# TinfoilHat0/Defending-Against-Backdoors-with-Robust-Learning-Rate

Measured on NVIDIA H100. Metric: fl_rounds_per_sec, higher is better.
Workload: dtype bf16

## Files before the change

defending-against-backdoors-with-robust-learning-rate_b200/models/native.py:

```python
from __future__ import annotations

import math
import os

import torch
import torch.nn.functional as F

from .. import ops
from .graph import FlatLayout

ACT = torch.bfloat16
FUSE_DROPOUT = bool(int(os.environ.get("RLR_FUSE_DROPOUT", "1")))
FUSE_RELU_POOL = bool(int(os.environ.get("RLR_FUSE_RELU_POOL", "1")))
EPILOGUE_BN_STATS = bool(int(os.environ.get("RLR_EPILOGUE_BN_STATS", "0")))
FWD_BRANCH = bool(int(os.environ.get("RLR_FWD_BRANCH", "1")))
BWD_BRANCH = bool(int(os.environ.get("RLR_BWD_BRANCH", "1")))
EPI_STAT_SLOTS = min(16, max(1, int(os.environ.get("RLR_EPI_STAT_SLOTS", "2"))))
FWD_SLOTS = BWD_SLOTS = max(1, int(os.environ.get("RLR_BN_SLOTS", "1")))
WGRAD_OVERLAP = bool(int(os.environ.get("RLR_WGRAD_OVERLAP", "1")))


def dropout_stream_base(seed: int, agent_id: int, rnd: int) -> int:
    z = (int(seed) * 0x9E3779B97F4A7C15 + (int(agent_id) + 1) * 0xBF58476D1CE4E5B9 + (int(rnd) + 1) * 0x94D049BB133111EB) & (2 ** 64 - 1)
    z = ((z ^ (z >> 30)) * 0xBF58476D1CE4E5B9) & (2 ** 64 - 1)
# ... 206 lines not shown
            op.saved["mean_rstd"] = torch.zeros(2, c, dtype=torch.float32, device=dev)
            off += 2 * c
        for op in self.plan:
            if op.kind == "gn":
                op.saved["mean_rstd"] = torch.zeros(B, 2, op.attrs["groups"], dtype=torch.float32, device=dev)
            if op.kind == "maxpool":
                op.saved["idx"] = torch.empty((B, *op.out_shape), dtype=torch.uint8, device=dev)
                if "drop" in op.saved and self.impl["pool"] != "sm100":
                    op.saved["dmask"] = torch.ones((B, *op.out_shape), dtype=torch.uint8, device=dev)
            if op.kind == "dropout":
                op.saved["mask"] = torch.empty((B, *op.out_shape), dtype=torch.uint8, device=dev)
        self._bn_src = {}
        for i, op in enumerate(self.plan):
            if not (FWD_BRANCH and op.kind == "conv" and ".downsample." in (op.name or "")):
                continue
            nxt = self.plan[i + 1] if i + 1 < len(self.plan) else None
            first = next((q for q in self.plan[:i] if q.x == op.x and q is not op), None)
            join = next((q for q in self.plan[i + 1:] if nxt is not None and q.res == nxt.y), None)
            if nxt is None or nxt.kind not in ("bn", "gn") or nxt.x != op.y or first is None or join is None:
                continue
            first.saved["fork_before"] = True
            op.saved["side_branch"] = nxt.saved["side_branch"] = True
            join.saved["join_before"] = True
        for i, op in enumerate(self.plan):
            if op.kind == "bn":
                prod = next((q for q in self.plan[:i] if q.y == op.x and q.kind == "conv"), None)
                op.saved["producer"] = prod

    def bind(self, w, wb, g, w_buffers=None):
        self.w, self.wb, self.g = w, wb, g
        lay = self.layout
        self.pw = {p.name: lay.view(w, p) for p in lay.params}
        self.pw.update({b.name: lay.view(w if w_buffers is None else w_buffers, b) for b in lay.buffers})
        self.pwb = {p.name: lay.view(wb, p) for p in lay.params} if wb is not None else {}
        self.pg = {p.name: lay.view(g, p) for p in lay.params} if g is not None else {}

    def T(self, t, B):
        return self.act[t][:B] if t != self.in_tid else self._x

    def stem_geometry(self):
        op = self.plan[0]
        if op.kind != "conv" or op.x != self.in_tid or self.impl["conv_fwd"] != "sm100" or self.impl["conv_wgrad"] != "sm100":
            return None
        return ops.stem_geometry(op.in_shape, op.attrs)

    def G(self, t, B):
# ... 92 lines not shown
        a = op.attrs
        x, y, dy = self.T(op.x, B), self.T(op.y, B), self.G(op.y, B)
        if op.relu and not op.saved.get("relu_bwd_fused"):
            ops.relu_bwd_(dy, y, self.impl["bn"])
        name = op.name + ".weight"
        gw, gb = self.pg[name], self.pg.get(op.name + ".bias")
        s, p = a.get("stride", 1), a.get("pad", 0)
        if self.impl["conv_wgrad"] == "sm100" and ops.conv_supported(op.in_shape, a, "wgrad"):
            if getattr(self, "_side", None) is not None:
                self._side.wait_stream(torch.cuda.current_stream(self.device))
                with torch.cuda.stream(self._side):
                    ops.conv2d_wgrad_sm100(x, dy, gw, gb, s, p, tag=(id(self), op.name), zero=False)
            else:
                ops.conv2d_wgrad_sm100(x, dy, gw, gb, s, p, tag=(id(self), op.name), zero=False)
        else:
            if self.impl["conv_wgrad"] == "sm100":
                ops.note_fallback("conv_wgrad", f"{op.name} in={op.in_shape} {a}")
            _, dw, db = torch.ops.aten.convolution_backward(
                dy.permute(0, 3, 1, 2), x.permute(0, 3, 1, 2), self.pwb[name].permute(0, 3, 1, 2),
                [a["cout"]] if gb is not None else None, [s, s], [p, p], [1, 1], False, [0, 0], 1, [False, True, gb is not None])
            gw.copy_(dw.permute(0, 2, 3, 1))
            if gb is not None:
                gb.copy_(db)
        if not op.need_dx:
            return
        dx = self.G(op.x, B)
        if self.impl["conv_dgrad"] == "sm100" and ops.conv_supported(op.in_shape, a, "dgrad"):
            ops.conv2d_dgrad_sm100(dy, self.pwb[name], dx, s, p, op.acc_dx)
            return
        if self.impl["conv_dgrad"] == "sm100":
            ops.note_fallback("conv_dgrad", f"{op.name} in={op.in_shape} {a}")
        di, _, _ = torch.ops.aten.convolution_backward(
            dy.permute(0, 3, 1, 2), x.permute(0, 3, 1, 2), self.pwb[name].permute(0, 3, 1, 2), None, [s, s], [p, p], [1, 1],
            False, [0, 0], 1, [True, False, False])
        di = di.permute(0, 2, 3, 1)
        if op.acc_dx:
            dx.add_(di)
        else:
            dx.copy_(di)

    def _fwd_bn(self, op, B, train):
        a = op.attrs
        x, y = self.T(op.x, B), self.T(op.y, B)
        res = self.T(op.res, B) if op.res is not None else None
        gamma, beta = self.pw[op.name + ".weight"], self.pw[op.name + ".bias"]
        rm, rv = self.pw[op.name + ".running_mean"], self.pw[op.name + ".running_var"]
        prod = op.saved["producer"]
        stats = prod.saved["stats"] if (train and prod is not None and prod.saved.get("stats_done")) else None
        if stats is not None and not self.fuse_bn_stats:
            stats = stats[0:EPI_STAT_SLOTS]
        count = x.numel() // x.shape[-1]
# ... 226 lines not shown
```

defending-against-backdoors-with-robust-learning-rate_b200/ops/__init__.py:

```python
from __future__ import annotations

import importlib.util
import os
import threading

import torch

_HERE = os.path.dirname(os.path.abspath(__file__))
_SO = os.path.join(_HERE, "_C.so")
_ext = None
_ext_err = None
_lock = threading.Lock()

MODE_IDS = {"avg": 0, "comed": 1, "sign": 2}
MAX_FUSED_AGENTS = 1024


class _Counter:
    calls = 0


class _CountingExt:
    def __init__(self, mod):
        self._mod = mod
# ... 356 lines not shown
        dl = dl.to(logits.dtype)
        if dlogits is not None:
            dlogits.copy_(dl)
            dl = dlogits
    if loss_sum is None:
        loss_sum = torch.zeros(1)
    loss_sum += loss
    if correct is not None:
        correct += (lf.argmax(1) == labels).sum().to(correct.dtype)
    return loss_sum, dl


def eval_metrics(logits, labels, loss_sum, confusion):
    if logits.is_cuda:
        ext().eval_metrics(logits.contiguous(), labels, loss_sum, confusion)
        return
    lf = logits.float()
    loss_sum += torch.nn.functional.cross_entropy(lf, labels, reduction="sum").double()
    C = lf.shape[1]
    pred = lf.argmax(1)
    confusion.view(-1).index_add_(0, labels * C + pred, torch.ones_like(labels))


from .nn import (avgpool_bwd, avgpool_fwd, bn_bwd, bn_fwd, conv2d_dgrad_sm100, conv2d_fwd_sm100, conv2d_wgrad_sm100, conv_supported,
                 dropout_bwd, dropout_fwd, gn_bwd, gn_fwd, linear_bwd, linear_fused_dropout_ok, linear_fwd, maxpool2_bwd, maxpool2_fwd, relu_bwd_, scratch, stem_geometry, STAT_SLOTS)
```

defending-against-backdoors-with-robust-learning-rate_b200/ops/csrc/gemm.cu:

```cuda
#include <cuda.h>
#include <stdlib.h>

#include "common.cuh"
#include "gemm.h"
#include "stem_gather.cuh"
#include "wgmma.cuh"

namespace rlr {

using namespace wg;

constexpr int BM = 128;
constexpr int BK = 64;
constexpr int kConsumers = 256;
constexpr int kThreads = kConsumers + 64;
constexpr int kEpiThreads = kConsumers;

template <int BN, int kOcc = 2>
struct TileCfg {
    static constexpr int kStages = kOcc == 3 ? (BN == 64 ? 3 : 2) : (BN == 64 ? 4 : 3);
    static constexpr int kABytes = BM * BK * 2;
    static constexpr int kBBytes = BN * BK * 2;
    static constexpr int kStageBytes = kABytes + kBBytes;
    static constexpr int kPitch = BN * 2 + 16;
// ... 246 lines not shown
                uint4 val = *reinterpret_cast<const uint4*>(staging + r * Cfg::kPitch + ch * 16);
                if (p.accumulate) {
                    const __nv_bfloat162* o2 = reinterpret_cast<const __nv_bfloat162*>(&oldv[j]);
                    __nv_bfloat162* v2 = reinterpret_cast<__nv_bfloat162*>(&val);
#pragma unroll
                    for (int q = 0; q < 4; ++q) {
                        const float2 a = __bfloat1622float2(v2[q]), b = __bfloat1622float2(o2[q]);
                        v2[q] = __floats2bfloat162_rn(a.x + b.x, a.y + b.y);
                    }
                }
                *reinterpret_cast<uint4*>(out + (size_t)gi * p.ldc + col0 + ch * 8) = val;
            }
        }
        if (kStats) {
            named_bar(1, kEpiThreads);
            for (int i = et; i < 2 * BN; i += kEpiThreads)
                if (col0 + (i % BN) < p.N)
                    atomicAdd(p.stats + (size_t)(blockIdx.x % kStatSlots) * 2 * p.N + (i < BN ? 0 : p.N) + col0 + (i % BN), red[i]);
        }
        }
    }
}

typedef CUresult (*EncodeTiledFn)(CUtensorMap*, CUtensorMapDataType, cuuint32_t, void*, const cuuint64_t*, const cuuint64_t*,
                                  const cuuint32_t*, const cuuint32_t*, CUtensorMapInterleave, CUtensorMapSwizzle,
                                  CUtensorMapL2promotion, CUtensorMapFloatOOBfill);

static EncodeTiledFn get_encode_fn() {
    static EncodeTiledFn fn = nullptr;
    if (!fn) {
        void* f = nullptr;
        cudaDriverEntryPointQueryResult q;
        if (cudaGetDriverEntryPoint("cuTensorMapEncodeTiled", &f, cudaEnableDefault, &q) != cudaSuccess || !f) return nullptr;
        fn = reinterpret_cast<EncodeTiledFn>(f);
    }
    return fn;
}

cudaError_t make_tmap_bf16(CUtensorMap* map, const void* base, int rank, const uint64_t* dims, const uint64_t* strides_bytes,
                           const uint32_t* box, const uint32_t* elem_strides = nullptr) {
    EncodeTiledFn fn = get_encode_fn();
    if (!fn) return cudaErrorNotSupported;
    cuuint64_t gd[5], gs[4];
    cuuint32_t bx[5], es[5];
    for (int i = 0; i < rank; ++i) {
        gd[i] = dims[i];
// ... 204 lines not shown
        const uint64_t d[4] = {(uint64_t)Cin, (uint64_t)Win, (uint64_t)Hin, (uint64_t)planes * NB};
        const uint64_t s[3] = {(uint64_t)Cin * 2, (uint64_t)Win * Cin * 2, (uint64_t)Hin * Win * Cin * 2};
        const uint32_t b[4] = {BK, (uint32_t)TW, (uint32_t)TH, (uint32_t)TN};
        const uint32_t es[4] = {1, (uint32_t)in_stride, (uint32_t)in_stride, 1};
        RLR_CUDA_CHECK(make_tmap_bf16(&tmA, x, 4, d, s, b, in_stride > 1 ? es : nullptr));
    }
    if (wtap) {
        if (bias) return cudaErrorInvalidValue;
        p.b_mn = 1; p.wcols = Cout;
        for (int t = 0; t < ntaps; ++t) p.wtap[t] = wtap[t];
        const uint64_t cols = (uint64_t)w_taps_total * Cout;
        const uint64_t d[2] = {cols, (uint64_t)Cin}, s[1] = {cols * 2};
        const uint32_t b[2] = {64, BK};
        RLR_CUDA_CHECK(make_tmap_bf16(&tmB, w, 2, d, s, b));
    } else {
        const uint64_t K = (uint64_t)ntaps * Cin;
        const uint64_t d[2] = {K, (uint64_t)Cout}, s[1] = {K * 2};
        const uint32_t b[2] = {BK, (uint32_t)bn};
        RLR_CUDA_CHECK(make_tmap_bf16(&tmB, w, 2, d, s, b));
    }
    return bn == 128 ? launch_bn<128>(tmA, tmB, p, m_tiles, st) : launch_bn<64>(tmA, tmB, p, m_tiles, st);
}

}
```

defending-against-backdoors-with-robust-learning-rate_b200/ops/csrc/gemm.h:

```cpp
#pragma once
#include <cuda_runtime.h>
#include <cuda_bf16.h>
#include <stdint.h>

#include "dropspec.h"

namespace rlr {

constexpr int kStatSlots = 16;

struct ConvGemmParams {
    int M, N, num_kb;
    int mode;
    int cblocks;
    int TW, TH, TN;
    int Ho, Wo, NB;
    int tiles_w, tiles_h;
    int ntaps;
    int in_stride;
    int out_stride, out_ph, out_pw, OutH, OutW;
    int8_t dh[9], dw[9];
    int dn[9];
    int b_mn;
    int wtap[9];
    int wcols;
    DropSpec drop;
    int tma_store;
    int split_prod;
    long long* dbg;
    const __nv_bfloat16* b_src;
    int b_ld, b_kvalid;
    const uint32_t* wait_flags;
    int wait_lo, wait_hi;
    const uint32_t* wait_epoch;
    void* out;
    int ldc;
    const float* bias;
    float* stats;
    int stat_slots;
    int relu, accumulate;
};

cudaError_t launch_gemm_bf16(const void* A, const void* B, void* out, int M, int N, int K, int lda, int ldb, int ldc,
                             const float* bias, int relu, int accumulate, float* stats, cudaStream_t st, const DropSpec* drop = nullptr);
cudaError_t launch_stem_gemm_bf16(const void* A, const void* W, void* out, int M, int N, int kvalid, int ldw, const float* bias, int relu,
                                  float* stats, const uint32_t* wait_flags, int wait_lo, int wait_hi, const uint32_t* wait_epoch,
                                  cudaStream_t st);
void set_pdl(int on);
cudaError_t launch_gemm_splitk_bf16(const void* A, const void* B, void* out, float* ws, int M, int N, int K, const float* bias, int relu,
                                    int num_sms, cudaStream_t st, const DropSpec* drop = nullptr);
void set_persistent_conv(int on);
void set_conv_occ3(int level);
void set_conv_tma_store(int on);
void set_conv_split_producer(int on);
void set_conv_trace(long long* buf);
long long* conv_trace_buf();
cudaError_t launch_conv_bf16(const void* x, const void* w, void* out, int NB, int planes, int Hin, int Win, int Cin, int Ho, int Wo,
                             int Cout, int ldc, int ntaps, const int* dh, const int* dw, const int* dplane, const float* bias,
                             int relu, int accumulate, float* stats, cudaStream_t st, const int* wtap = nullptr, int w_taps_total = 0,
                             int in_stride = 1, int out_stride = 1, int out_ph = 0, int out_pw = 0);

cudaError_t launch_conv3x3_halo_bf16(const void* x, const void* w, void* out, int NB, int Hin, int Win, int H, int W, int Cout, const float* bias,
                                     int relu, int accumulate, float* stats, int bo_mode, long long* dbg, int num_sms, cudaStream_t st);

cudaError_t launch_conv3x3_halo3_bf16(const void* x, const void* w, void* out, int NB, int H, int W, int Cout, const float* bias, int relu,
                                      int accumulate, int num_sms, cudaStream_t st);

cudaError_t launch_conv_wgrad_bf16(const void* dy, const void* x, float* dW, int NB, int planes, int Hin, int Win, int Cin, int Cin_valid,
                                   int Ho, int Wo, int Cout, int ntaps, const int* dh, const int* dw, const int* dplane, int num_sms,
                                   cudaStream_t st, int in_stride = 1);
cudaError_t launch_conv_wgrad_halo_bf16(const void* dy, const void* x, float* dW, int NB, int H, int W, int Cin_valid, int Cout,
                                        int num_sms, cudaStream_t st);
cudaError_t launch_linear_wgrad_bf16(const void* dy, const void* x, float* dW, int B, int N, int K, int num_sms, cudaStream_t st);

cudaError_t launch_ordered_sum_f32(float* out, const float* part, int nparts, long long n, cudaStream_t st);
cudaError_t launch_ordered_sum_f64(double* out, const double* part, int nparts, long long n, cudaStream_t st);
cudaError_t launch_channel_stats(const __nv_bfloat16* x, long long M, int C, float* stats , int num_sms, cudaStream_t st,
                                 int only_sum = 0, int nslots = 1);
cudaError_t launch_bn_finalize(const float* stats, int slots, float* mean_rstd, float* running_mean, float* running_var, int C,
                               float count, float eps, float momentum, int train, cudaStream_t st);
cudaError_t launch_bn_apply(const __nv_bfloat16* x, const __nv_bfloat16* res, __nv_bfloat16* y, const float* gamma, const float* beta,
                            float* mean_rstd, long long M, int C, int relu, int fin_mode, const float* stats, int slots, float count,
                            float eps, float momentum, float* running_mean, float* running_var, int num_sms, cudaStream_t st);
// ... 40 lines not shown
```

defending-against-backdoors-with-robust-learning-rate_b200/ops/csrc/gemm_binding.cpp:

```cpp
#include <torch/extension.h>
#include <ATen/cuda/CUDAContext.h>
#include <c10/cuda/CUDAGuard.h>
#include <c10/cuda/CUDAStream.h>
#include <c10/cuda/CUDACachingAllocator.h>

#include <vector>

#include "gemm.h"

namespace rlr {
void* scratch_alloc(size_t bytes, cudaStream_t st) {
    return c10::cuda::CUDACachingAllocator::raw_alloc_with_stream(bytes < 256 ? 256 : bytes, st);
}
void scratch_free(void* p) { c10::cuda::CUDACachingAllocator::raw_delete(p); }
}

namespace {
inline cudaStream_t cur_stream() { return c10::cuda::getCurrentCUDAStream().stream(); }
inline int num_sms() { return at::cuda::getCurrentDeviceProperties()->multiProcessorCount; }
inline void check(cudaError_t e, const char* what) { TORCH_CHECK(e == cudaSuccess, what, ": ", cudaGetErrorString(e)); }
template <typename T>
inline T* opt(const c10::optional<at::Tensor>& t) { return t.has_value() && t->defined() ? reinterpret_cast<T*>(t->data_ptr()) : nullptr; }
inline const __nv_bfloat16* bf(const at::Tensor& t) {
    TORCH_CHECK(t.is_cuda() && t.scalar_type() == at::kBFloat16 && t.is_contiguous(), "expected contiguous CUDA bf16 tensor");
// ... 64 lines not shown
    const int M = A.size(0), K = A.size(1), N = B.size(0);
    TORCH_CHECK(B.size(1) == K && out.size(0) == M && out.size(1) == N && ws.numel() == (int64_t)M * N);
    check(rlr::launch_gemm_splitk_bf16(bf(A), bf(B), bfm(out), f32(ws), M, N, K, opt<const float>(bias), relu, num_sms(), cur_stream(),
                                       drop.thr ? &drop : nullptr), "gemm_splitk_bf16");
}

void conv_bf16_strided(at::Tensor x, at::Tensor w, at::Tensor out, std::vector<int64_t> dh, std::vector<int64_t> dw,
                       c10::optional<at::Tensor> bias, bool relu, bool accumulate, std::vector<int64_t> wtap, int64_t w_taps_total,
                       int64_t in_stride, int64_t out_stride, int64_t out_ph, int64_t out_pw) {
    c10::cuda::CUDAGuard g(x.device());
    TORCH_CHECK(x.dim() == 4 && out.dim() == 4 && w.dim() == 2 && x.size(0) == out.size(0));
    TORCH_CHECK(out.size(1) % out_stride == 0 && out.size(2) % out_stride == 0, "output image must be a multiple of out_stride");
    const int NB = x.size(0), Hin = x.size(1), Win = x.size(2), Cin = x.size(3), Cout = out.size(3);
    const int Ho = out.size(1) / out_stride, Wo = out.size(2) / out_stride;
    const int T = (int)dh.size();
    const bool bmn = !wtap.empty();
    TORCH_CHECK(bmn ? (w.size(0) == Cin && w.size(1) == w_taps_total * Cout && (int)wtap.size() == T)
                    : (w.size(0) == Cout && w.size(1) == (int64_t)T * Cin), "filter shape");
    int a[9], b[9], c[9] = {0}, wt[9];
    for (int t = 0; t < T; ++t) { a[t] = (int)dh[t]; b[t] = (int)dw[t]; wt[t] = bmn ? (int)wtap[t] : 0; }
    check(rlr::launch_conv_bf16(bf(x), bf(w), bfm(out), NB, 1, Hin, Win, Cin, Ho, Wo, Cout, Cout, T, a, b, c, opt<const float>(bias), relu,
                                accumulate, nullptr, cur_stream(), bmn ? wt : nullptr, (int)w_taps_total, (int)in_stride, (int)out_stride,
                                (int)out_ph, (int)out_pw), "conv_bf16_strided");
}

void conv3x3_halo_bf16(at::Tensor x, at::Tensor w, at::Tensor out, c10::optional<at::Tensor> bias, bool relu, bool accumulate,
                       c10::optional<at::Tensor> stats, int64_t bo_mode, c10::optional<at::Tensor> dbg) {
    c10::cuda::CUDAGuard g(x.device());
    TORCH_CHECK(x.dim() == 4 && x.size(3) == 64 && out.dim() == 4 && w.dim() == 2 && w.size(1) == 9 * 64 && w.size(0) == out.size(3));
    TORCH_CHECK(out.size(0) == x.size(0) && out.size(1) - x.size(1) == out.size(2) - x.size(2), "halo conv: output = input + 2*pad - 2, pad in {0,1,2}");
    TORCH_CHECK(!stats.has_value() || !stats->defined() || stats->numel() == (int64_t)rlr::kStatSlots * 2 * out.size(3), "stats must be [STAT_SLOTS,2,Cout]");
    check(rlr::launch_conv3x3_halo_bf16(bf(x), bf(w), bfm(out), x.size(0), x.size(1), x.size(2), out.size(1), out.size(2), out.size(3), opt<const float>(bias), relu,
                                        accumulate, opt<float>(stats), (int)bo_mode, opt<long long>(dbg), num_sms(), cur_stream()), "conv3x3_halo_bf16");
}

void conv3x3_halo3_bf16(at::Tensor x, at::Tensor w, at::Tensor out, c10::optional<at::Tensor> bias, bool relu, bool accumulate) {
    c10::cuda::CUDAGuard g(x.device());
    TORCH_CHECK(x.dim() == 4 && x.size(3) == 64 && out.dim() == 4 && w.dim() == 2 && w.size(1) == 9 * 64 && w.size(0) == out.size(3));
    TORCH_CHECK(out.size(0) == x.size(0) && out.size(1) == x.size(1) && out.size(2) == x.size(2));
    check(rlr::launch_conv3x3_halo3_bf16(bf(x), bf(w), bfm(out), x.size(0), x.size(1), x.size(2), out.size(3), opt<const float>(bias), relu,
                                         accumulate, num_sms(), cur_stream()), "conv3x3_halo3_bf16");
}

void conv_wgrad_bf16(at::Tensor dy, at::Tensor x, at::Tensor dW, int64_t NB, int64_t planes, int64_t cin_valid, std::vector<int64_t> dh,
                     std::vector<int64_t> dw, std::vector<int64_t> dplane) {
    c10::cuda::CUDAGuard g(x.device());
// ... 216 lines not shown
    check(rlr::launch_linear_small_bwd2(bf(x), bf(dy), bf(w), const_cast<__nv_bfloat16*>(bfo(dx)), (float*)dw.data_ptr(), opt<float>(db),
                                        x.size(0), x.size(1), w.size(0), accumulate_dx, cur_stream()), "linear_small_bwd2");
}
}

void register_gemm_bindings(py::module_& m) {
    m.attr("STAT_SLOTS") = rlr::kStatSlots;
    m.def("set_persistent_conv", [](bool on) { rlr::set_persistent_conv(on ? 1 : 0); });
    m.def("set_pdl", [](bool on) { rlr::set_pdl(on ? 1 : 0); });
    m.def("set_conv_occ3", [](int64_t level) { rlr::set_conv_occ3((int)level); });
    m.def("set_conv_tma_store", [](bool on) { rlr::set_conv_tma_store(on ? 1 : 0); });
    m.def("set_conv_split_producer", [](bool on) { rlr::set_conv_split_producer(on ? 1 : 0); });
    m.def("set_conv_trace", [](c10::optional<at::Tensor> buf) {
        rlr::set_conv_trace(buf.has_value() && buf->defined() ? reinterpret_cast<long long*>(buf->data_ptr<int64_t>()) : nullptr);
    });
    m.def("gemm_bf16", &gemm_bf16, py::arg("A"), py::arg("B"), py::arg("out"), py::arg("bias"), py::arg("relu"), py::arg("accumulate"), py::arg("stats"),
          py::arg("drop_p") = 0.0, py::arg("drop_seed") = 0, py::arg("drop_step") = py::none(), py::arg("drop_stream") = 0);
    m.def("stem_gemm_bf16", &stem_gemm_bf16, py::arg("A"), py::arg("W"), py::arg("out"), py::arg("bias"), py::arg("relu"), py::arg("stats"),
          py::arg("ready_ptr") = 0, py::arg("lo") = 0, py::arg("hi") = 0, py::arg("epoch") = py::none());
    m.def("gemm_splitk_bf16", &gemm_splitk_bf16, py::arg("A"), py::arg("B"), py::arg("out"), py::arg("ws"), py::arg("bias"), py::arg("relu"),
          py::arg("drop_p") = 0.0, py::arg("drop_seed") = 0, py::arg("drop_step") = py::none(), py::arg("drop_stream") = 0);
    m.def("conv_bf16", &conv_bf16);
    m.def("conv_bf16_strided", &conv_bf16_strided);
    m.def("conv_wgrad_bf16_strided", &conv_wgrad_bf16_strided);
    m.def("conv3x3_halo_bf16", &conv3x3_halo_bf16);
    m.def("conv3x3_halo3_bf16", &conv3x3_halo3_bf16);
    m.def("conv_wgrad_bf16", &conv_wgrad_bf16);
    m.def("linear_wgrad_bf16", &linear_wgrad_bf16);
    m.def("conv_wgrad_halo_bf16", &conv_wgrad_halo_bf16);
    m.def("channel_stats", &channel_stats);
    m.def("ordered_sum", &ordered_sum);
    m.def("bias_grad", &bias_grad);
    m.def("bn_finalize", &bn_finalize);
    m.def("bn_apply", &bn_apply);
    m.def("bn_bwd", &bn_bwd);
    m.def("bn_bwd_recompute", &bn_bwd_recompute);
    m.def("gn_fwd", &gn_fwd);
    m.def("gn_bwd", &gn_bwd);
    m.def("relu_bwd", &relu_bwd, py::arg("dy"), py::arg("y"), py::arg("scale") = 1.0);
    m.def("maxpool2_fwd", &maxpool2_fwd, py::arg("x"), py::arg("y"), py::arg("idx"), py::arg("drop_p") = 0.0, py::arg("drop_seed") = 0,
          py::arg("drop_step") = py::none(), py::arg("drop_stream") = 0);
    m.def("maxpool2_bwd", &maxpool2_bwd, py::arg("dy"), py::arg("idx"), py::arg("dx"), py::arg("drop_p") = 0.0, py::arg("drop_seed") = 0,
          py::arg("drop_step") = py::none(), py::arg("drop_stream") = 0, py::arg("relu_out") = py::none());
    m.def("avgpool_fwd", &avgpool_fwd);
    m.def("avgpool_bwd", &avgpool_bwd);
    m.def("dropout_fwd", &dropout_fwd);
// ... 12 lines not shown
```

defending-against-backdoors-with-robust-learning-rate_b200/ops/nn.py:

```python
from __future__ import annotations

import math
import os

import torch
import torch.nn.functional as F

_scratch = {}
_s2d_done = {}
STAT_SLOTS = 16
USE_WGRAD_HALO = True
USE_STRIDED_TMA = bool(int(os.environ.get("RLR_STRIDED_TMA", "1")))
USE_IM2COL_STEM = bool(int(os.environ.get("RLR_IM2COL_STEM", "1")))
USE_BN_RECOMPUTE = bool(int(os.environ.get("RLR_BN_RECOMPUTE", "1")))
USE_HALO3 = bool(int(os.environ.get("RLR_HALO3", "0")))
USE_HALO_ANY = bool(int(os.environ.get("RLR_HALO_ANY", "1")))
USE_SPLITK = bool(int(os.environ.get("RLR_SPLITK", "1")))
USE_HEAD_V2 = bool(int(os.environ.get("RLR_HEAD_V2", "1")))


def _stem_ok(k, stride, cin, cout):
    return USE_IM2COL_STEM and stride == 1 and cin * k * k <= 64 and cout % 8 == 0 and (cout <= 64 or cout % 128 == 0)


def stem_geometry(in_shape, a):
    h, w, c = in_shape
    k, s, p = a["k"], a.get("stride", 1), a.get("pad", 0)
    if not _stem_ok(k, s, c, a["cout"]):
        return None
    return k, p, h + 2 * p - k + 1, w + 2 * p - k + 1


def _ext():
    from . import ext
    return ext()
# ... 121 lines not shown
    B = dy.shape[0]
    if stride == 2:
        return _conv2d_dgrad_s2(e, dy, w, dx, pad, accumulate)
    if _halo_ok(k, 1, k - 1 - pad, Cout, dy.shape[1], dy.shape[2]) and dx.shape[-1] % 8 == 0:
        wt = scratch(("wt", w.data_ptr(), dx.data_ptr()), (Cin, k * k * Cout), w.dtype, w.device)
        e.filter_transpose(w, wt, Cout, k * k, Cin)
        if USE_HALO3 and pad == 1 and dy.shape[1] % 16 == 0:
            e.conv3x3_halo3_bf16(dy, wt, dx, None, False, bool(accumulate))
        else:
            e.conv3x3_halo_bf16(dy, wt, dx, None, False, bool(accumulate), None, 0, None)
        return dx
    dh, dw, pl = _taps(k, 1, k - 1 - pad)
    if Cin % 64 == 0:
        T = k * k
        e.conv_bf16(dy, w.reshape(Cout, T * Cin), dx, B, 1, dh, dw, pl, None, False, bool(accumulate), None,
                    [T - 1 - t for t in range(T)], T)
        return dx
    wt = scratch(("wt", w.data_ptr(), dx.data_ptr()), (Cin, k * k * Cout), w.dtype, w.device)
    e.filter_transpose(w, wt, Cout, k * k, Cin)
    e.conv_bf16(dy, wt, dx, B, 1, dh, dw, pl, None, False, bool(accumulate), None, [], 0)
    return dx


def _conv2d_dgrad_s2(e, dy, w, dx, pad, accumulate):
    Cout, k, _, Cin = w.shape
    B, Ho, Wo, _ = dy.shape
    plan = []
    for pi in range(2):
        for pj in range(2):
            taps, dh, dw = [], [], []
            for fy in range(k):
                for fx in range(k):
                    if (pi + pad - fy) % 2 == 0 and (pj + pad - fx) % 2 == 0:
                        taps.append(fy * k + fx); dh.append((pi + pad - fy) // 2); dw.append((pj + pad - fx) // 2)
            if taps:
                plan.append((pi, pj, taps, dh, dw))
    if USE_STRIDED_TMA and Cin % 64 == 0 and dx.shape[1] == 2 * Ho and dx.shape[2] == 2 * Wo:
        if not accumulate and len(plan) < 4:
            _zero(dx)
        for pi, pj, taps, dh, dw in plan:
            e.conv_bf16_strided(dy, w.reshape(Cout, k * k * Cin), dx, dh, dw, None, False, bool(accumulate), taps, k * k, 1, 2, pi, pj)
        return dx
    dx4 = scratch(("dx4", w.data_ptr(), dx.data_ptr()), (4 * B, Ho, Wo, Cin), dy.dtype, dy.device)
    mask = 0
    for pi, pj, taps, dh, dw in plan:
        plane = pi * 2 + pj
        mask |= 1 << plane
        if Cin % 64 == 0:
            e.conv_bf16(dy, w.reshape(Cout, k * k * Cin), dx4[plane * B:(plane + 1) * B], B, 1, dh, dw, [0] * len(taps), None,
                        False, False, None, taps, k * k)
            continue
        wt = scratch(("wt_s2", w.data_ptr(), dx.data_ptr(), plane), (Cin, len(taps) * Cout), w.dtype, w.device)
        e.filter_gather_transpose(w, wt, Cout, k * k, Cin, taps)
        e.conv_bf16(dy, wt, dx4[plane * B:(plane + 1) * B], B, 1, dh, dw, [0] * len(taps), None, False, False, None, [], 0)
    e.depth_to_space(dx4, dx, bool(accumulate), mask)
    return dx


def conv2d_wgrad_sm100(x, dy, gw, gb, stride, pad, tag="fwd", zero=True):
# ... 323 lines not shown
```

Baseline: 0.5344.

## Fuse stride-2 dgrad planes and downsample shortcut dgrad into one kernel

Adds a single-launch UMMA kernel that computes all four output parity planes of a stride-2 conv dgrad at once, instead of one launch per plane plus a zeroing pass. For ResNet downsample blocks, the 1x1 stride-2 shortcut conv's dgrad is folded into the main conv's kernel as extra K-blocks on the (0,0) plane, so the separate shortcut launch and its read-modify-write accumulation disappear. The plan builder marks these pairs and skips the shortcut's own dgrad. The cost is added complexity, tensor map setup per call, and a shortcut partial that is rounded to bf16 before it is summed in.

```diff
diff --git a/defending-against-backdoors-with-robust-learning-rate_b200/models/native.py b/defending-against-backdoors-with-robust-learning-rate_b200/models/native.py
--- a/defending-against-backdoors-with-robust-learning-rate_b200/models/native.py
+++ b/defending-against-backdoors-with-robust-learning-rate_b200/models/native.py
@@ -252,6 +252,20 @@
             first.saved["fork_before"] = True
             op.saved["side_branch"] = nxt.saved["side_branch"] = True
             join.saved["join_before"] = True
+        if self.impl["conv_dgrad"] == "sm100" and ops.nn.USE_FUSED_S2_DGRAD and ops.nn.USE_STRIDED_TMA:
+            for i, op in enumerate(self.plan):
+                if not (op.kind == "conv" and ".downsample." in (op.name or "")) or not op.need_dx or op.acc_dx or op.relu:
+                    continue
+                first = next((q for q in self.plan[:i] if q.kind == "conv" and q.x == op.x), None)
+                writers = [q for q in self.plan if q.x == op.x or q.res == op.x]
+                a = op.attrs
+                if (first is None or len(writers) != 2 or (a["k"], a.get("stride", 1), a.get("pad", 0)) != (1, 2, 0)
+                        or first.attrs.get("stride", 1) != 2 or first.attrs["cout"] != a["cout"]
+                        or not ops.conv_supported(first.in_shape, first.attrs, "dgrad") or not ops.conv_supported(op.in_shape, a, "dgrad")):
+                    continue
+                first.saved["dgrad_shortcut"] = op
+                op.saved["dgrad_folded"] = True
+                first.acc_dx = False
         for i, op in enumerate(self.plan):
             if op.kind == "bn":
                 prod = next((q for q in self.plan[:i] if q.y == op.x and q.kind == "conv"), None)
@@ -390,11 +404,15 @@
             gw.copy_(dw.permute(0, 2, 3, 1))
             if gb is not None:
                 gb.copy_(db)
-        if not op.need_dx:
+        if not op.need_dx or op.saved.get("dgrad_folded"):
             return
         dx = self.G(op.x, B)
         if self.impl["conv_dgrad"] == "sm100" and ops.conv_supported(op.in_shape, a, "dgrad"):
-            ops.conv2d_dgrad_sm100(dy, self.pwb[name], dx, s, p, op.acc_dx)
+            sc = op.saved.get("dgrad_shortcut")
+            if sc is not None:
+                ops.conv2d_dgrad_s2_fused(dy, self.pwb[name], dx, p, op.acc_dx, self.G(sc.y, B), self.pwb[sc.name + ".weight"])
+            else:
+                ops.conv2d_dgrad_sm100(dy, self.pwb[name], dx, s, p, op.acc_dx)
             return
         if self.impl["conv_dgrad"] == "sm100":
             ops.note_fallback("conv_dgrad", f"{op.name} in={op.in_shape} {a}")
diff --git a/defending-against-backdoors-with-robust-learning-rate_b200/ops/__init__.py b/defending-against-backdoors-with-robust-learning-rate_b200/ops/__init__.py
--- a/defending-against-backdoors-with-robust-learning-rate_b200/ops/__init__.py
+++ b/defending-against-backdoors-with-robust-learning-rate_b200/ops/__init__.py
@@ -402,5 +402,5 @@
     confusion.view(-1).index_add_(0, labels * C + pred, torch.ones_like(labels))
 
 
-from .nn import (avgpool_bwd, avgpool_fwd, bn_bwd, bn_fwd, conv2d_dgrad_sm100, conv2d_fwd_sm100, conv2d_wgrad_sm100, conv_supported,
+from .nn import (avgpool_bwd, avgpool_fwd, bn_bwd, bn_fwd, conv2d_dgrad_s2_fused, conv2d_dgrad_sm100, conv2d_fwd_sm100, conv2d_wgrad_sm100, conv_supported,
                  dropout_bwd, dropout_fwd, gn_bwd, gn_fwd, linear_bwd, linear_fused_dropout_ok, linear_fwd, maxpool2_bwd, maxpool2_fwd, relu_bwd_, scratch, stem_geometry, STAT_SLOTS)
diff --git a/defending-against-backdoors-with-robust-learning-rate_b200/ops/csrc/gemm.cu b/defending-against-backdoors-with-robust-learning-rate_b200/ops/csrc/gemm.cu
--- a/defending-against-backdoors-with-robust-learning-rate_b200/ops/csrc/gemm.cu
+++ b/defending-against-backdoors-with-robust-learning-rate_b200/ops/csrc/gemm.cu
@@ -1,5 +1,6 @@
 #include <cuda.h>
 #include <stdlib.h>
+#include <string.h>
 
 #include "common.cuh"
 #include "gemm.h"
@@ -292,6 +293,178 @@
     }
 }
 
+struct S2DgradMaps {
+    CUtensorMap a_sc, b_sc;
+    CUtensorMap c[4];
+};
+
+template <int BN>
+__global__ void __launch_bounds__(kThreads, 3)
+umma_dgrad_s2_kernel(const __grid_constant__ CUtensorMap tmA, const __grid_constant__ CUtensorMap tmB, const __grid_constant__ S2DgradMaps mp,
+                     const ConvGemmParams p) {
+    using Cfg = TileCfg<BN, 3>;
+    extern __shared__ uint8_t smem_raw[];
+    uint8_t* smem = reinterpret_cast<uint8_t*>((reinterpret_cast<uintptr_t>(smem_raw) + 1023) & ~uintptr_t(1023));
+    SharedTail* tail = reinterpret_cast<SharedTail*>(smem + Cfg::kRingBytes);
+
+    const int warp = threadIdx.x >> 5, lane = threadIdx.x & 31;
+    const auto tile_of = [&](int& slot, int& tile_n, int& w0, int& h0, int& n0) {
+        slot = blockIdx.x / p.plane_ctas;
+        const int rem = blockIdx.x - slot * p.plane_ctas;
+        tile_n = rem / p.m_tiles;
+        const int tile_m = rem - tile_n * p.m_tiles;
+        w0 = (tile_m % p.tiles_w) * p.TW; h0 = ((tile_m / p.tiles_w) % p.tiles_h) * p.TH; n0 = (tile_m / (p.tiles_w * p.tiles_h)) * p.TN;
+    };
+    int slot, tile_n, w0, h0, n0;
+    tile_of(slot, tile_n, w0, h0, n0);
+    const int tap0 = p.pl_tap0[slot], ph = p.pl_ph[slot], pw = p.pl_pw[slot];
+    const int sc_kb = slot == p.sc_slot ? p.cblocks : 0;
+    const int main_kb = p.pl_ntaps[slot] * p.cblocks;
+    const int num_kb = sc_kb + main_kb;
+
+    if (warp == 8 && lane == 0) {
+        prefetch_tmap(&tmA);
+        prefetch_tmap(&tmB);
+        if (p.tma_store) prefetch_tmap(&mp.c[slot]);
+        if (sc_kb) { prefetch_tmap(&mp.a_sc); prefetch_tmap(&mp.b_sc); }
+        for (int s = 0; s < Cfg::kStages; ++s) { mbar_init(&tail->full[s], 2); mbar_init(&tail->empty[s], 8); }
+        fence_barrier_init();
+    }
+    if (threadIdx.x < BM) {
+        const int r = threadIdx.x;
+        const int w = w0 + r % p.TW, h = h0 + (r / p.TW) % p.TH, n = n0 + r / (p.TW * p.TH);
+        tail->row_index[r] = (w < p.Wo && h < p.Ho && n < p.NB) ? ((n * p.OutH + 2 * h + ph) * p.OutW + 2 * w + pw) : -1;
+    }
+    __syncthreads();
+    pdl_wait();
+    pdl_trigger();
+
+    if (warp == 8) {
+        if (lane == 0) {
+            int stage = 0;
+            uint32_t phase = 0;
+            for (int kb = 0; kb < num_kb; ++kb) {
+                mbar_wait(&tail->empty[stage], phase ^ 1);
+                uint8_t* sa = smem + stage * Cfg::kStageBytes;
+                mbar_expect_tx(&tail->full[stage], Cfg::kABytes);
+                if (kb < sc_kb) {
+                    tma_load_4d(&mp.a_sc, &tail->full[stage], sa, kb * BK, w0, h0, n0);
+                } else {
+                    const int i = kb - sc_kb, tap = tap0 + i / p.cblocks, cb = i % p.cblocks;
+                    tma_load_4d(&tmA, &tail->full[stage], sa, cb * BK, w0 + p.dw[tap], h0 + p.dh[tap], n0);
+                }
+                if (++stage == Cfg::kStages) { stage = 0; phase ^= 1; }
+            }
+        }
+    } else if (warp == 9) {
+        if (lane == 0) {
+            int stage = 0;
+            uint32_t phase = 0;
+            for (int kb = 0; kb < num_kb; ++kb) {
+                mbar_wait(&tail->empty[stage], phase ^ 1);
+                uint8_t* sb = smem + stage * Cfg::kStageBytes + Cfg::kABytes;
+                mbar_expect_tx(&tail->full[stage], Cfg::kBBytes);
+                if (kb < sc_kb) {
+#pragma unroll
+                    for (int g = 0; g < BN / 64; ++g) tma_load_2d(&mp.b_sc, &tail->full[stage], sb + g * 8192, tile_n * BN + g * 64, kb * BK);
+                } else {
+                    const int i = kb - sc_kb, tap = tap0 + i / p.cblocks, cb = i % p.cblocks;
+#pragma unroll
+                    for (int g = 0; g < BN / 64; ++g)
+                        tma_load_2d(&tmB, &tail->full[stage], sb + g * 8192, p.wtap[tap] * p.wcols + tile_n * BN + g * 64, cb * BK);
+                }
+                if (++stage == Cfg::kStages) { stage = 0; phase ^= 1; }
+            }
+        }
+    } else {
+        const int et = threadIdx.x;
+        const int wgi = et >> 7;
+        float acc[BN / 2];
+        uint32_t sc[BN / 4];
+#pragma unroll
+        for (int i = 0; i < BN / 2; ++i) acc[i] = 0.f;
+#pragma unroll
+        for (int i = 0; i < BN / 4; ++i) sc[i] = 0u;
+        int stage = 0;
+        uint32_t phase = 0;
+        if (sc_kb) {
+            consumer_mainloop<BN, Cfg::kStages, Cfg::kStageBytes, Cfg::kABytes, true>(acc, smem, tail->full, tail->empty, sc_kb,
+                                                                                     (uint32_t)wgi * 64 * 128, 0u, stage, phase, lane);
+#pragma unroll
+            for (int i = 0; i < BN / 4; ++i) { sc[i] = pack_bf16x2(acc[2 * i], acc[2 * i + 1]); acc[2 * i] = acc[2 * i + 1] = 0.f; }
+        }
+        consumer_mainloop<BN, Cfg::kStages, Cfg::kStageBytes, Cfg::kABytes, true>(acc, smem, tail->full, tail->empty, main_kb,
+                                                                                 (uint32_t)wgi * 64 * 128, 0u, stage, phase, lane);
+        named_bar(1, kEpiThreads);
+        tile_of(slot, tile_n, w0, h0, n0);
+        const int t = et & 127, col0 = tile_n * BN;
+        uint8_t* staging = smem;
+        const int r0 = wgi * 64 + frag_row(t, 0);
+        const bool tma_out = p.tma_store;
+#pragma unroll
+        for (int j = 0; j < BN / 8; ++j) {
+            const int c = frag_col(t, 4 * j);
+#pragma unroll
+            for (int h = 0; h < 2; ++h) {
+                const int row = r0 + 8 * h;
+                uint32_t packed = pack_bf16x2(acc[4 * j + 2 * h], acc[4 * j + 2 * h + 1]);
+                if (p.sc_round) {
+                    const float2 m = __bfloat1622float2(*reinterpret_cast<const __nv_bfloat162*>(&packed));
+                    const float2 s = __bfloat1622float2(*reinterpret_cast<const __nv_bfloat162*>(&sc[2 * j + h]));
+                    packed = pack_bf16x2(m.x + s.x, m.y + s.y);
+                }
+                if (tma_out)
+                    *reinterpret_cast<uint32_t*>(staging + (c >> 6) * (BM * 128) + row * 128 + ((((c & 63) >> 3) ^ (row & 7)) << 4) + (c & 7) * 2) = packed;
+                else
+                    *reinterpret_cast<uint32_t*>(staging + row * Cfg::kPitch + c * 2) = packed;
+            }
+        }
+        if (tma_out) {
+            fence_proxy_async_smem();
+            named_bar(1, kEpiThreads);
+            if (et == 0) {
+#pragma unroll
+                for (int g = 0; g < BN / 64; ++g) {
+                    if (col0 + g * 64 >= p.N) break;
+                    tma_store_4d(&mp.c[slot], staging + g * (BM * 128), col0 + g * 64, w0, h0, n0);
+                }
+                tma_store_commit();
+                tma_store_wait_read();
+            }
+        } else {
+            named_bar(1, kEpiThreads);
+            constexpr int kChunks = BN * 2 / 16;
+            constexpr int kIters = BM * kChunks / kEpiThreads;
+            __nv_bfloat16* out = reinterpret_cast<__nv_bfloat16*>(p.out);
+            uint4 oldv[kIters];
+#pragma unroll
+            for (int j = 0; j < kIters; ++j) {
+                const int idx = et + j * kEpiThreads, r = idx / kChunks, ch = idx - r * kChunks;
+                const int gi = tail->row_index[r];
+                oldv[j] = make_uint4(0, 0, 0, 0);
+                if (p.accumulate && gi >= 0 && col0 + ch * 8 < p.N) oldv[j] = *reinterpret_cast<const uint4*>(out + (size_t)gi * p.ldc + col0 + ch * 8);
+            }
+#pragma unroll
+            for (int j = 0; j < kIters; ++j) {
+                const int idx = et + j * kEpiThreads, r = idx / kChunks, ch = idx - r * kChunks;
+                const int gi = tail->row_index[r];
+                if (gi < 0 || col0 + ch * 8 >= p.N) continue;
+                uint4 val = *reinterpret_cast<const uint4*>(staging + r * Cfg::kPitch + ch * 16);
+                if (p.accumulate) {
+                    const __nv_bfloat162* o2 = reinterpret_cast<const __nv_bfloat162*>(&oldv[j]);
+                    __nv_bfloat162* v2 = reinterpret_cast<__nv_bfloat162*>(&val);
+#pragma unroll
+                    for (int q = 0; q < 4; ++q) {
+                        const float2 a = __bfloat1622float2(v2[q]), b = __bfloat1622float2(o2[q]);
+                        v2[q] = __floats2bfloat162_rn(a.x + b.x, a.y + b.y);
+                    }
+                }
+                *reinterpret_cast<uint4*>(out + (size_t)gi * p.ldc + col0 + ch * 8) = val;
+            }
+        }
+    }
+}
+
 typedef CUresult (*EncodeTiledFn)(CUtensorMap*, CUtensorMapDataType, cuuint32_t, void*, const cuuint64_t*, const cuuint64_t*,
                                   const cuuint32_t*, const cuuint32_t*, CUtensorMapInterleave, CUtensorMapSwizzle,
                                   CUtensorMapL2promotion, CUtensorMapFloatOOBfill);
@@ -542,4 +715,78 @@
     return bn == 128 ? launch_bn<128>(tmA, tmB, p, m_tiles, st) : launch_bn<64>(tmA, tmB, p, m_tiles, st);
 }
 
-}
+cudaError_t launch_conv_dgrad_s2_bf16(const void* dy, const void* w, void* dx, int NB, int Ho, int Wo, int K, int Cin, int w_taps_total,
+                                      const int* dh, const int* dw, const int* wtap, int nplanes, const int* plane_ph, const int* plane_pw,
+                                      const int* plane_ntaps, const void* dy_sc, const void* w_sc, int accumulate, cudaStream_t st) {
+    constexpr int BN = 64;
+    using Cfg = TileCfg<BN, 3>;
+    if (K % BK || Cin % BN || NB < 1 || Ho < 1 || Wo < 1 || nplanes < 1 || nplanes > 4 || w_taps_total < 1) return cudaErrorInvalidValue;
+    if ((dy_sc == nullptr) != (w_sc == nullptr) || (dy_sc && accumulate)) return cudaErrorInvalidValue;
+    ConvGemmParams p{};
+    int TW = pow2_ceil(Wo); if (TW > BM) TW = BM;
+    int TH = pow2_ceil(Ho); if (TW * TH > BM) TH = BM / TW;
+    p.TW = TW; p.TH = TH; p.TN = BM / (TW * TH);
+    p.tiles_w = (Wo + TW - 1) / TW; p.tiles_h = (Ho + TH - 1) / TH;
+    p.m_tiles = p.tiles_w * p.tiles_h * ((NB + p.TN - 1) / p.TN);
+    p.plane_ctas = p.m_tiles * (Cin / BN);
+    p.M = NB * Ho * Wo; p.N = Cin; p.mode = 1; p.cblocks = K / BK; p.Ho = Ho; p.Wo = Wo; p.NB = NB;
+    p.in_stride = 1; p.out_stride = 2; p.OutH = 2 * Ho; p.OutW = 2 * Wo;
+    p.b_mn = 1; p.wcols = Cin; p.out = dx; p.ldc = Cin; p.accumulate = accumulate;
+    int tap0[4], order[4], kbs[4], ntot = 0, sc_plane = -1;
+    for (int i = 0; i < nplanes; ++i) {
+        if (plane_ntaps[i] < 0 || (plane_ph[i] & ~1) || (plane_pw[i] & ~1)) return cudaErrorInvalidValue;
+        tap0[i] = ntot; ntot += plane_ntaps[i];
+        if (dy_sc && plane_ph[i] == 0 && plane_pw[i] == 0) sc_plane = i;
+        kbs[i] = plane_ntaps[i] + (i == sc_plane);
+        order[i] = i;
+    }
+    if (ntot > 9 || (dy_sc && sc_plane < 0)) return cudaErrorInvalidValue;
+    for (int i = 1; i < nplanes; ++i)
+        for (int j = i; j > 0 && kbs[order[j]] > kbs[order[j - 1]]; --j) { const int o = order[j]; order[j] = order[j - 1]; order[j - 1] = o; }
+    for (int t = 0; t < ntot; ++t) {
+        if (wtap[t] < 0 || wtap[t] >= w_taps_total) return cudaErrorInvalidValue;
+        p.dh[t] = (int8_t)dh[t]; p.dw[t] = (int8_t)dw[t]; p.wtap[t] = wtap[t];
+    }
+    p.sc_slot = -1;
+    p.sc_round = dy_sc != nullptr;
+    p.tma_store = tma_store_enabled() && !accumulate && (reinterpret_cast<uintptr_t>(dx) & 15) == 0;
+    CUtensorMap tmA, tmB;
+    S2DgradMaps mp;
+    memset(&mp, 0, sizeof(mp));
+    {
+        const uint64_t d[4] = {(uint64_t)K, (uint64_t)Wo, (uint64_t)Ho, (uint64_t)NB};
+        const uint64_t s[3] = {(uint64_t)K * 2, (uint64_t)Wo * K * 2, (uint64_t)Ho * Wo * K * 2};
+        const uint32_t b[4] = {BK, (uint32_t)TW, (uint32_t)TH, (uint32_t)p.TN};
+        RLR_CUDA_CHECK(make_tmap_bf16(&tmA, dy, 4, d, s, b));
+        if (dy_sc) RLR_CUDA_CHECK(make_tmap_bf16(&mp.a_sc, dy_sc, 4, d, s, b));
+    }
+    {
+        const uint64_t cols = (uint64_t)w_taps_total * Cin;
+        const uint64_t d[2] = {cols, (uint64_t)K}, s[1] = {cols * 2};
+        const uint32_t b[2] = {64, BK};
+        RLR_CUDA_CHECK(make_tmap_bf16(&tmB, w, 2, d, s, b));
+        if (w_sc) {
+            const uint64_t d1[2] = {(uint64_t)Cin, (uint64_t)K}, s1[1] = {(uint64_t)Cin * 2};
+            RLR_CUDA_CHECK(make_tmap_bf16(&mp.b_sc, w_sc, 2, d1, s1, b));
+        }
+    }
+    for (int sl = 0; sl < nplanes; ++sl) {
+        const int i = order[sl];
+        p.pl_tap0[sl] = (int8_t)tap0[i]; p.pl_ntaps[sl] = (int8_t)plane_ntaps[i];
+        p.pl_ph[sl] = (int8_t)plane_ph[i]; p.pl_pw[sl] = (int8_t)plane_pw[i];
+        if (i == sc_plane) p.sc_slot = sl;
+        if (p.tma_store) {
+            p.out_ph = plane_ph[i]; p.out_pw = plane_pw[i];
+            RLR_CUDA_CHECK(make_out_tmap(&mp.c[sl], p));
+        }
+    }
+    p.out_ph = p.out_pw = 0;
+    static bool configured = false;
+    if (!configured) {
+        RLR_CUDA_CHECK(cudaFuncSetAttribute(umma_dgrad_s2_kernel<BN>, cudaFuncAttributeMaxDynamicSharedMemorySize, Cfg::kSmemBytes));
+        configured = true;
+    }
+    return launch_kernel(umma_dgrad_s2_kernel<BN>, dim3(nplanes * p.plane_ctas), dim3(kThreads), Cfg::kSmemBytes, st, tmA, tmB, mp, p);
+}
+
+}
diff --git a/defending-against-backdoors-with-robust-learning-rate_b200/ops/csrc/gemm.h b/defending-against-backdoors-with-robust-learning-rate_b200/ops/csrc/gemm.h
--- a/defending-against-backdoors-with-robust-learning-rate_b200/ops/csrc/gemm.h
+++ b/defending-against-backdoors-with-robust-learning-rate_b200/ops/csrc/gemm.h
@@ -39,6 +39,8 @@
     float* stats;
     int stat_slots;
     int relu, accumulate;
+    int m_tiles, plane_ctas, sc_slot, sc_round;
+    int8_t pl_tap0[4], pl_ntaps[4], pl_ph[4], pl_pw[4];
 };
 
 cudaError_t launch_gemm_bf16(const void* A, const void* B, void* out, int M, int N, int K, int lda, int ldb, int ldc,
@@ -59,6 +61,9 @@
                              int Cout, int ldc, int ntaps, const int* dh, const int* dw, const int* dplane, const float* bias,
                              int relu, int accumulate, float* stats, cudaStream_t st, const int* wtap = nullptr, int w_taps_total = 0,
                              int in_stride = 1, int out_stride = 1, int out_ph = 0, int out_pw = 0);
+cudaError_t launch_conv_dgrad_s2_bf16(const void* dy, const void* w, void* dx, int NB, int Ho, int Wo, int K, int Cin, int w_taps_total,
+                                      const int* dh, const int* dw, const int* wtap, int nplanes, const int* plane_ph, const int* plane_pw,
+                                      const int* plane_ntaps, const void* dy_sc, const void* w_sc, int accumulate, cudaStream_t st);
 
 cudaError_t launch_conv3x3_halo_bf16(const void* x, const void* w, void* out, int NB, int Hin, int Win, int H, int W, int Cout, const float* bias,
                                      int relu, int accumulate, float* stats, int bo_mode, long long* dbg, int num_sms, cudaStream_t st);
diff --git a/defending-against-backdoors-with-robust-learning-rate_b200/ops/csrc/gemm_binding.cpp b/defending-against-backdoors-with-robust-learning-rate_b200/ops/csrc/gemm_binding.cpp
--- a/defending-against-backdoors-with-robust-learning-rate_b200/ops/csrc/gemm_binding.cpp
+++ b/defending-against-backdoors-with-robust-learning-rate_b200/ops/csrc/gemm_binding.cpp
@@ -110,6 +110,29 @@
     check(rlr::launch_conv_bf16(bf(x), bf(w), bfm(out), NB, 1, Hin, Win, Cin, Ho, Wo, Cout, Cout, T, a, b, c, opt<const float>(bias), relu,
                                 accumulate, nullptr, cur_stream(), bmn ? wt : nullptr, (int)w_taps_total, (int)in_stride, (int)out_stride,
                                 (int)out_ph, (int)out_pw), "conv_bf16_strided");
+}
+
+void conv_dgrad_s2_fused(at::Tensor dy, at::Tensor w, at::Tensor dx, std::vector<int64_t> dh, std::vector<int64_t> dw,
+                         std::vector<int64_t> wtap, int64_t w_taps_total, std::vector<int64_t> plane_ph, std::vector<int64_t> plane_pw,
+                         std::vector<int64_t> plane_ntaps, bool accumulate, c10::optional<at::Tensor> dy_sc, c10::optional<at::Tensor> w_sc) {
+    c10::cuda::CUDAGuard g(dy.device());
+    TORCH_CHECK(dy.dim() == 4 && dx.dim() == 4 && w.dim() == 2 && dy.size(0) == dx.size(0), "conv_dgrad_s2_fused shapes");
+    const int NB = dy.size(0), Ho = dy.size(1), Wo = dy.size(2), K = dy.size(3), Cin = dx.size(3);
+    TORCH_CHECK(dx.size(1) == 2 * Ho && dx.size(2) == 2 * Wo, "dx must be exactly 2Ho x 2Wo");
+    TORCH_CHECK(w.size(0) == K && w.size(1) == w_taps_total * Cin, "filter shape");
+    const int T = (int)dh.size(), P = (int)plane_ph.size();
+    TORCH_CHECK(T <= 9 && (int)dw.size() == T && (int)wtap.size() == T && P >= 1 && P <= 4 && (int)plane_pw.size() == P &&
+                (int)plane_ntaps.size() == P, "tap / plane tables");
+    const bool sc = dy_sc.has_value() && dy_sc->defined();
+    TORCH_CHECK(sc == (w_sc.has_value() && w_sc->defined()), "dy_sc and w_sc go together");
+    if (sc) TORCH_CHECK(dy_sc->sizes() == dy.sizes() && w_sc->dim() == 2 && w_sc->size(0) == K && w_sc->size(1) == Cin, "shortcut shapes");
+    int a[9], b[9], wt[9], pph[4], ppw[4], pnt[4], sum = 0;
+    for (int t = 0; t < T; ++t) { a[t] = (int)dh[t]; b[t] = (int)dw[t]; wt[t] = (int)wtap[t]; }
+    for (int i = 0; i < P; ++i) { pph[i] = (int)plane_ph[i]; ppw[i] = (int)plane_pw[i]; pnt[i] = (int)plane_ntaps[i]; sum += pnt[i]; }
+    TORCH_CHECK(sum == T, "plane tap counts must add up to the tap table");
+    check(rlr::launch_conv_dgrad_s2_bf16(bf(dy), bf(w), bfm(dx), NB, Ho, Wo, K, Cin, (int)w_taps_total, a, b, wt, P, pph, ppw, pnt,
+                                         sc ? bf(*dy_sc) : nullptr, sc ? bf(*w_sc) : nullptr, accumulate, cur_stream()),
+          "conv_dgrad_s2_fused");
 }
 
 void conv3x3_halo_bf16(at::Tensor x, at::Tensor w, at::Tensor out, c10::optional<at::Tensor> bias, bool relu, bool accumulate,
@@ -372,6 +395,7 @@
           py::arg("drop_p") = 0.0, py::arg("drop_seed") = 0, py::arg("drop_step") = py::none(), py::arg("drop_stream") = 0);
     m.def("conv_bf16", &conv_bf16);
     m.def("conv_bf16_strided", &conv_bf16_strided);
+    m.def("conv_dgrad_s2_fused", &conv_dgrad_s2_fused);
     m.def("conv_wgrad_bf16_strided", &conv_wgrad_bf16_strided);
     m.def("conv3x3_halo_bf16", &conv3x3_halo_bf16);
     m.def("conv3x3_halo3_bf16", &conv3x3_halo3_bf16);
diff --git a/defending-against-backdoors-with-robust-learning-rate_b200/ops/nn.py b/defending-against-backdoors-with-robust-learning-rate_b200/ops/nn.py
--- a/defending-against-backdoors-with-robust-learning-rate_b200/ops/nn.py
+++ b/defending-against-backdoors-with-robust-learning-rate_b200/ops/nn.py
@@ -11,6 +11,7 @@
 STAT_SLOTS = 16
 USE_WGRAD_HALO = True
 USE_STRIDED_TMA = bool(int(os.environ.get("RLR_STRIDED_TMA", "1")))
+USE_FUSED_S2_DGRAD = bool(int(os.environ.get("RLR_FUSED_S2_DGRAD", "1")))
 USE_IM2COL_STEM = bool(int(os.environ.get("RLR_IM2COL_STEM", "1")))
 USE_BN_RECOMPUTE = bool(int(os.environ.get("RLR_BN_RECOMPUTE", "1")))
 USE_HALO3 = bool(int(os.environ.get("RLR_HALO3", "0")))
@@ -178,9 +179,7 @@
     return dx
 
 
-def _conv2d_dgrad_s2(e, dy, w, dx, pad, accumulate):
-    Cout, k, _, Cin = w.shape
-    B, Ho, Wo, _ = dy.shape
+def _s2_planes(k, pad):
     plan = []
     for pi in range(2):
         for pj in range(2):
@@ -189,8 +188,55 @@
                 for fx in range(k):
                     if (pi + pad - fy) % 2 == 0 and (pj + pad - fx) % 2 == 0:
                         taps.append(fy * k + fx); dh.append((pi + pad - fy) // 2); dw.append((pj + pad - fx) // 2)
-            if taps:
-                plan.append((pi, pj, taps, dh, dw))
+            plan.append((pi, pj, taps, dh, dw))
+    return plan
+
+
+def _fused_s2_ok(e, Cin, dx, dy):
+    return (USE_FUSED_S2_DGRAD and USE_STRIDED_TMA and Cin % 64 == 0 and dx.shape[1] == 2 * dy.shape[1] and dx.shape[2] == 2 * dy.shape[2]
+            and hasattr(e, "conv_dgrad_s2_fused"))
+
+
+def _dgrad_s2_one_launch(e, dy, w, dx, pad, accumulate, dy_sc, w_sc):
+    Cout, k, _, Cin = w.shape
+    plan = _s2_planes(k, pad)
+    if accumulate:
+        plan = [q for q in plan if q[2]]
+    e.conv_dgrad_s2_fused(dy, w.reshape(Cout, k * k * Cin), dx, [d for q in plan for d in q[3]], [d for q in plan for d in q[4]],
+                          [t for q in plan for t in q[2]], k * k, [q[0] for q in plan], [q[1] for q in plan], [len(q[2]) for q in plan],
+                          bool(accumulate), dy_sc, w_sc.reshape(Cout, Cin) if w_sc is not None else None)
+    return dx
+
+
+def conv2d_dgrad_s2_fused(dy, w, dx, pad, accumulate, dy_sc=None, w_sc=None, impl="sm100"):
+    if dy_sc is not None and accumulate:
+        raise ValueError("conv2d_dgrad_s2_fused: a shortcut gradient is only folded into a first write of dx")
+    if impl == "aten":
+        def dgrad(g, wt, p):
+            return torch.ops.aten.convolution_backward(g.permute(0, 3, 1, 2), dx.permute(0, 3, 1, 2), wt.permute(0, 3, 1, 2), None, [2, 2],
+                                                       [p, p], [1, 1], False, [0, 0], 1, [True, False, False])[0].permute(0, 2, 3, 1)
+        r = dgrad(dy, w, pad).to(dx.dtype)
+        if dy_sc is not None:
+            r = r.float() + dgrad(dy_sc, w_sc, 0).to(dx.dtype).float()
+        if accumulate:
+            r = r.float() + dx.float()
+        dx.copy_(r)
+        return dx
+    e = _ext()
+    if _fused_s2_ok(e, w.shape[3], dx, dy):
+        return _dgrad_s2_one_launch(e, dy, w, dx, pad, accumulate, dy_sc, w_sc)
+    if dy_sc is not None:
+        _conv2d_dgrad_s2(e, dy_sc, w_sc, dx, 0, False)
+        accumulate = True
+    return _conv2d_dgrad_s2(e, dy, w, dx, pad, accumulate)
+
+
+def _conv2d_dgrad_s2(e, dy, w, dx, pad, accumulate):
+    Cout, k, _, Cin = w.shape
+    B, Ho, Wo, _ = dy.shape
+    if _fused_s2_ok(e, Cin, dx, dy):
+        return _dgrad_s2_one_launch(e, dy, w, dx, pad, accumulate, None, None)
+    plan = [q for q in _s2_planes(k, pad) if q[2]]
     if USE_STRIDED_TMA and Cin % 64 == 0 and dx.shape[1] == 2 * Ho and dx.shape[2] == 2 * Wo:
         if not accumulate and len(plan) < 4:
             _zero(dx)
```

Result: faster. 0.5450, median of 6 (+2.0%).
